# ChicyChen/LOCO-Edit

Measured on AMD Instinct MI355X. Metric: edit-directions/sec (top-5 PMP-Jacobian SVD @256^2) + vT cos-sim vs ref, higher is better.
Workload: dtype bf16x3 (split-bf16 MFMA operands, fp32 accumulate + fp32 storage); 1 GPU; CelebA-HQ DDPM 256x256 top-5 local basis (l_eye-sized mask, L=2400), t=0.6T, 12 power iterations, one GPU; multi_gpu_form=single, probes_total=5, probes_per_gpu=5, kept=5, n_iter=12, mask_L=2400, weights=synthetic seed 0, streams=2

## Files before the change

### loco-edit_amd/csrc/conv_bf16_kernel.h

```cpp
#pragma once
#include "kernels.h"
#include <cstdlib>
#include <type_traits>

namespace loco {


typedef float f32x16 __attribute__((ext_vector_type(16)));
typedef float f32x4 __attribute__((ext_vector_type(4)));
typedef f32x4 f32x4_u __attribute__((aligned(4)));
typedef float f32x2 __attribute__((ext_vector_type(2)));
typedef f32x2 f32x2_u __attribute__((aligned(4)));
typedef __bf16 bf16x8 __attribute__((ext_vector_type(8)));
typedef _Float16 f16x8 __attribute__((ext_vector_type(8)));
typedef short s16x8 __attribute__((ext_vector_type(8)));

enum : int { PR_BF16X3 = 0, PR_F16 = 1 };

constexpr int BKC = 16;
constexpr bool LIVE_MASK = true;
constexpr bool EARLY_W = true;
constexpr int NDUMMY = 8;

__device__ __forceinline__ float sigmoidf2_(float y) { return __builtin_amdgcn_rcpf(1.0f + __expf(-y)); }
// ... 46 lines not shown
    if (taps == 1) return NT;
    if (NT >= 128) {
        int th = NT / 32;
        return s2 ? (2 * th + 1) * 65 : (th + 2) * 34;
    }
    return s2 ? 5 * 65 : 4 * 34;
}

constexpr int rs_steps(int n, int lw) { int s = 0; while ((1 << s) < lw && (n >> s) > 1) ++s; return s; }
template <int N, int M, int LW>
__device__ __forceinline__ void rs_reduce(float* av, const int lane) {
    if constexpr (M < LW && N > 1) {
        constexpr int H = N / 2;
        const bool up = (lane & M) != 0;
#pragma unroll
        for (int i = 0; i < H; ++i) {
            const float keep = up ? av[i + H] : av[i];
            const float send = up ? av[i] : av[i + H];
            av[i] = keep + __shfl_xor(send, M, 64);
        }
        rs_reduce<H, M * 2, LW>(av, lane);
    } else if constexpr (M < LW) {
#pragma unroll
        for (int i = 0; i < N; ++i) av[i] += __shfl_xor(av[i], M, 64);
        rs_reduce<N, M * 2, LW>(av, lane);
    }
}

constexpr int EPI_COT1 = 1, EPI_STATS = 2;
template <int WM, int WN, int TM, int TN, int EPI = EPI_STATS, class StageRound>
__device__ __forceinline__ void conv_lowp_epilogue_staged(const ConvArgs& a, StageRound&& stage_round, unsigned char* smem_b, const int co0,
                                                          const int oy0, const int ox0, const int TW, const int tile_id, const int b,
                                                          const int split);
template <int WM, int WN, int TM, int TN>
__device__ __forceinline__ void conv_lowp_epilogue_direct(const ConvArgs& a, f32x16 (&acc)[TM][TN], const int co0, const int oy0,
                                                          const int ox0, const int TW, const int b, const int split);
template <int WM, int WN, int TM, int TN, int EPI = EPI_STATS>
__device__ __forceinline__ void conv_lowp_epilogue(const ConvArgs& a, f32x16 (&acc)[TM][TN], unsigned char* smem_b, const int co0,
                                                   const int oy0, const int ox0, const int TW, const int tile_id, const int b,
                                                   const int split) {
    constexpr int NT = WN * TN * 32;
    const int lane = threadIdx.x & 63, wave = threadIdx.x >> 6;
    const int l31 = lane & 31, khalf = lane >> 5, wm = wave / WN, wn = wave % WN;
    if (co0 + WM * TM * 32 <= a.Cout) {
        conv_lowp_epilogue_staged<WM, WN, TM, TN, EPI>(a, [&](const int h, float* S) {
#pragma unroll
            for (int j = 0; j < TN; ++j)
#pragma unroll
                for (int r = 0; r < 16; ++r)
                    S[(wm * 32 + (r & 3) + 8 * (r >> 2) + 4 * khalf) * NT + (wn * TN + j) * 32 + l31] = acc[h][j][r];
        }, smem_b, co0, oy0, ox0, TW, tile_id, b, split);
        return;
    }
    conv_lowp_epilogue_direct<WM, WN, TM, TN>(a, acc, co0, oy0, ox0, TW, b, split);
}
template <int WM, int WN, int TM, int TN, int EPI, class StageRound>
__device__ __forceinline__ void conv_lowp_epilogue_staged(const ConvArgs& a, StageRound&& stage_round, unsigned char* smem_b, const int co0,
                                                          const int oy0, const int ox0, const int TW, const int tile_id, const int b,
                                                          const int split) {
    constexpr int NTHR = WM * WN * 64;
    constexpr bool COT1 = (EPI & EPI_COT1) != 0, STATS = (EPI & EPI_STATS) != 0;
    constexpr int MT = WM * TM * 32;
    constexpr int NT = WN * TN * 32;
    const int tid = threadIdx.x;
    const int lane = tid & 63;
    const int wave = tid >> 6;
    const int l31 = lane & 31;
    const int khalf = lane >> 5;
    const int wm = wave / WN, wn = wave % WN;
    const long out_plane = (long)a.Hout * a.Wout;
    {
        constexpr int SROWS = WM * 32, NQ = NT / 4, NTASK = (SROWS * NQ) / NTHR;
        static_assert((SROWS * NQ) % NTHR == 0 && (NQ & (NQ - 1)) == 0, "epilogue task split");
        float* const S = reinterpret_cast<float*>(smem_b);
        const bool part = a.nsplit > 1;
        float* const ob = part ? a.partial + (((long)split * a.B + b) * a.Cout) * out_plane : a.out + (long)b * a.out_bs;
        const float* const rb = (!part && a.res) ? a.res + (long)b * a.res_bs : nullptr;
        const float* const b2 = (!part && a.bias2) ? a.bias2 + (long)b * a.bias2_bs : nullptr;
        const float* const b1 = part ? nullptr : a.bias;
        const bool accu = !part && a.accumulate;
        const int twsh = 31 - __builtin_clz((unsigned)TW);
        const bool lin_st = STATS && (a.st_kind == ST_TAN || a.st_kind == ST_COT) && !part;
        const bool lin_cot = a.st_kind == ST_COT;
        const bool cot_ep = COT1 && a.cot_d && !part && !lin_st;
        const float* const cot_db = cot_ep ? a.cot_d + (long)b * a.cot_d_bs : nullptr;
        const f32x2* const cot_tb = cot_ep ? reinterpret_cast<const f32x2*>(a.cot_tc + (long)b * a.cot_tc_bs) : nullptr;
        constexpr int RSTEP = NTHR / NQ;
// ... 110 lines not shown
                        s1 += __shfl_xor(s1, m, 64);
                        s2 += __shfl_xor(s2, m, 64);
                    }
                    const float m = s1 * (1.0f / NT);
                    const int t = q * NTHR + tid;
                    if ((t & (NQ - 1)) == 0)
                        *reinterpret_cast<f32x2*>(sp + ((long)co_of(h, q) * ntile + tile_id) * 2) = f32x2{pivot + m, s2 - s1 * m};
                }
            }
        }
        if constexpr (STATS) if (lin_st) {
            constexpr int LW = NQ < 64 ? NQ : 64, STEPS = rs_steps(NV, LW), LEFT = NV >> STEPS;
            static_assert((NV & (NV - 1)) == 0, "row sums per lane");
            rs_reduce<NV, 1, LW>(av, lane);
            const int gl = lane & (LW - 1);
            if (gl < (1 << STEPS)) {
                int base = 0;
#pragma unroll
                for (int sb = 0; sb < STEPS; ++sb) base += ((gl >> sb) & 1) * (NV >> (sb + 1));
                const int ntile = (a.Hout * a.Wout) / NT;
                float* const sp = a.st_part + (long)b * a.Cout * ntile * 2;
#pragma unroll
                for (int i = 0; i < LEFT; ++i) {
                    const int idx = base + i, hq = idx >> 1;
                    const int h = hq / NTASK, q = hq - h * NTASK;
                    const int row = (q * NTHR + tid) / NQ;
                    const int co = co0 + ((row >> 5) * TM + h) * 32 + (row & 31);
                    sp[((long)co * ntile + tile_id) * 2 + (idx & 1)] = av[i];
                }
            }
        }
    }
}
template <int WM, int WN, int TM, int TN>
__device__ __forceinline__ void conv_lowp_epilogue_direct(const ConvArgs& a, f32x16 (&acc)[TM][TN], const int co0, const int oy0,
                                                          const int ox0, const int TW, const int b, const int split) {
    const int lane = threadIdx.x & 63, wave = threadIdx.x >> 6;
    const int l31 = lane & 31, khalf = lane >> 5, wm = wave / WN, wn = wave % WN;
    const long out_plane = (long)a.Hout * a.Wout;
    const bool full_co = false;
#pragma unroll
    for (int j = 0; j < TN; ++j) {
        int p = (wn * TN + j) * 32 + l31;
        int ty = p / TW, tx = p - ty * TW;
        int oy = oy0 + ty, ox = ox0 + tx;
        const unsigned pix = (unsigned)(oy * a.Wout + ox);
#pragma unroll
        for (int i = 0; i < TM; ++i) {
            const int cob = co0 + (wm * TM + i) * 32 + 4 * khalf;
            if (a.nsplit > 1) {
                float* pb = a.partial + (((long)split * a.B + b) * a.Cout) * out_plane;
#pragma unroll
                for (int r = 0; r < 16; ++r) {
                    int co = cob + (r & 3) + 8 * (r >> 2);
                    if (full_co || co < a.Cout) pb[(long)co * out_plane + pix] = acc[i][j][r];
                }
            } else {
                float* ob = a.out + (long)b * a.out_bs;
                const float* rb = a.res ? a.res + (long)b * a.res_bs : nullptr;
                const float* b2 = a.bias2 ? a.bias2 + (long)b * a.bias2_bs : nullptr;
                if (rb || a.accumulate) {
                    float rv[16];
#pragma unroll
                    for (int r = 0; r < 16; ++r) {
                        int co = cob + (r & 3) + 8 * (r >> 2);
                        const bool ok = full_co || co < a.Cout;
                        const long off = (long)(ok ? co : a.Cout - 1) * out_plane + pix;
                        float t = 0.f;
                        if (rb) t = a.res_scale * rb[off];
                        if (a.accumulate) t += ob[off];
                        rv[r] = t;
                    }
#pragma unroll
                    for (int r = 0; r < 16; ++r) {
                        int co = cob + (r & 3) + 8 * (r >> 2);
                        if (!(full_co || co < a.Cout)) continue;
// ... 1 lines not shown
                        if (a.bias) v += a.bias[co];
                        if (b2) v += b2[co];
                        __builtin_nontemporal_store(v, &ob[(long)co * out_plane + pix]);
                    }
                } else {
#pragma unroll
                    for (int r = 0; r < 16; ++r) {
                        int co = cob + (r & 3) + 8 * (r >> 2);
                        if (!(full_co || co < a.Cout)) continue;
                        float v = acc[i][j][r];
                        if (a.bias) v += a.bias[co];
                        if (b2) v += b2[co];
                        __builtin_nontemporal_store(v, &ob[(long)co * out_plane + pix]);
                    }
                }
            }
        }
    }
}

template <int PR, int TAPS, int WM, int WN, int TM, int TN, int MODE, int STG, int PHASE = 0>
__device__ __forceinline__ void conv_lowp_body(const ConvArgs& a, f32x16 (&acc)[TM][TN]) {
    constexpr int NTHR = WM * WN * 64;
    constexpr int HP = halo_pitch<PR>();
    constexpr int RB = rec_bytes<PR>();
    constexpr int NPC = RB / 16;
    constexpr int MT = WM * TM * 32;
    constexpr int NT = WN * TN * 32;
    constexpr int KS = (TAPS == 9) ? 3 : 1;
    constexpr int NTS = KS;
    constexpr int NROW = (TAPS == 9) ? 3 : 1;
    constexpr bool NEEDP = (MODE == CM_TAN_SILU || MODE == CM_COT_SILU);
    constexpr bool GEN = (STG == 1 || STG == 2);
    constexpr int NITEM = GEN ? (2 * max_halo(NT, TAPS, STG == 2) + NTHR - 1) / NTHR : 1;
    constexpr int WTOT = NTS * MT * NPC;
    constexpr int NWV = (WTOT + NTHR - 1) / NTHR;
    constexpr bool XPF = (TAPS == 9 && STG != 2);
    constexpr int NWB = XPF ? 3 : 2;
    constexpr bool DEEP1 = (TAPS == 1 && STG == 1 && !NEEDP);
    constexpr int DEEP_D = 4;

    extern __shared__ __attribute__((aligned(16))) unsigned char smem_b[];
#ifdef LOCO_DUAL_STAMP
#define LP_STAMP(i) do { if (threadIdx.x == 0 && PHASE == 0) reinterpret_cast<unsigned long long*>(a.partial)[blockIdx.x * 8 + (i)] = __builtin_amdgcn_s_memtime(); } while (0)
#else
#define LP_STAMP(i) do { } while (0)
#endif
    LP_STAMP(0);
    constexpr int WBYTES = NTS * MT * RB;
    unsigned char* const Wsb = smem_b;
    unsigned char* Hsb;
    unsigned char* Ws = smem_b;
    unsigned char* Hs = smem_b;

    const int tid = threadIdx.x;
    const int lane = tid & 63;
    const int wave = tid >> 6;
    const int l31 = lane & 31;
    const int khalf = lane >> 5;
    const int wm = wave / WN, wn = wave % WN;

    const int S = a.stride;
    const int TW = (TAPS == 1 && PHASE == 0 && a.stride == 1 && !a.upsample && !a.zins && (a.Wout & (a.Wout - 1)) == 0)
                       ? (a.Wout < NT ? a.Wout : NT) : (a.Wout < 32 ? a.Wout : 32);
    const int TH = NT / TW;
    const int tiles_x = a.Wout / TW;
// ... 23 lines not shown
    const int co0 = cot_id * MT;
    int zb_, zs_;
    idivmod_small(zid, a.nsplit, zb_, zs_);
    const int b = __builtin_amdgcn_readfirstlane(zb_);
    const int split = __builtin_amdgcn_readfirstlane(zs_);

    if constexpr (XPF && PHASE != 2 && EARLY_W) {
        const int nchunks_ = (a.Cin + BKC - 1) / BKC;
        const int cps_ = __builtin_amdgcn_readfirstlane((nchunks_ + a.nsplit - 1) / a.nsplit);
        const int cbeg_ = split * cps_;
        const int cend_ = (cbeg_ + cps_ < nchunks_) ? cbeg_ + cps_ : nchunks_;
        if (cend_ > cbeg_) {
            typedef __attribute__((address_space(3))) unsigned char lds_u8_;
            typedef const __attribute__((address_space(1))) unsigned char glb_u8_;
            const int wpitch_ = (a.Cout + 31) & ~31;
            const unsigned char* wbase0 = reinterpret_cast<const unsigned char*>(a.wb) +
                                          (unsigned)(cbeg_ * TAPS) * ((unsigned)wpitch_ * (unsigned)RB);
#pragma unroll
            for (int st_ = 0; st_ < 2; ++st_)
#pragma unroll
                for (int i = 0; i < NWV; ++i) {
                    int e = tid + i * NTHR;
                    if (e >= WTOT) e = WTOT - 1;
                    const int tap = e / (MT * NPC), rem = e - tap * (MT * NPC);
                    int rec = co0 + rem / NPC;
                    if (rec >= wpitch_) rec = wpitch_ - 1;
                    const unsigned rel = (unsigned)(((st_ * NTS + tap) * wpitch_ + rec) * NPC + (rem % NPC)) * 16u;
                    const int e0 = wave * 64 + i * NTHR;
                    if ((WTOT % NTHR) == 0 || e0 < WTOT)
                        __builtin_amdgcn_global_load_lds((glb_u8_*)(wbase0 + rel), (lds_u8_*)(smem_b + st_ * WBYTES + e0 * 16), 16, 0, 0);
                }
        }
    }
    const int halo_w = (TW - 1) * S + KS;
    const int halo_h = (TH - 1) * S + KS;
    const int halo_sz = halo_h * halo_w;
    const int HBYTES = (halo_sz + NDUMMY) * HP;
    Hsb = smem_b + NWB * WBYTES;

    const int LH = (a.upsample || a.zins) ? a.Hin * 2 : a.Hin;
    const int LW = (a.upsample || a.zins) ? a.Win * 2 : a.Win;
    const long in_plane = (long)a.Hin * a.Win;

    int ipos[NITEM], ioct[NITEM];
    unsigned ivoff[NITEM];
    bool ival[NITEM];
#pragma unroll
    for (int i = 0; i < NITEM; ++i) {
        int it = tid + i * NTHR;
        int oct, pos;
        idivmod_small(it, halo_sz, oct, pos);
        int off = -1;
        if (it < 2 * halo_sz) {
            int hy, hx;
            idivmod_small(pos, halo_w, hy, hx);
            int Y = oy0 * S - a.pad + hy, X = ox0 * S - a.pad + hx;
            if (Y >= 0 && Y < LH && X >= 0 && X < LW) {
                if (a.upsample) off = (Y >> 1) * a.Win + (X >> 1);
                else if (a.zins) off = ((Y | X) & 1) ? -1 : (Y >> 1) * a.Win + (X >> 1);
                else off = Y * a.Win + X;
            }
        } else {
            pos = -1; oct = 0;
        }
        ipos[i] = pos; ioct[i] = oct;
        ival[i] = off >= 0;
        ivoff[i] = (unsigned)(oct * 8 * (int)in_plane + (off >= 0 ? off : 0));
    }

    const int nseg = (halo_w + 3) >> 2;
    int v_q4 = 0, v_pos0 = -1, v_voff = 0, v_cnt = 0;
    unsigned v_pm = 0;
    int v_rec[4] = {0, 0, 0, 0};
    unsigned v_goff = 0;
    if constexpr (!GEN) {
        const int per_q = halo_h * nseg;
        const int nsg4 = (nseg + 3) >> 2, nhy2 = (halo_h + 1) >> 1;
        bool have = false;
        int hy = 0, sg = 0;
        if (32 * nsg4 * nhy2 <= NTHR) {
            const int hi = tid >> 5;
            v_q4 = (tid >> 3) & 3;
            int hq_, hr_;
            idivmod_small(hi, nsg4, hq_, hr_);
            sg = hr_ * 4 + (tid & 3);
            hy = hq_ * 2 + ((tid >> 2) & 1);
            have = hi < nsg4 * nhy2 && sg < nseg && hy < halo_h;
            if (!have) v_q4 = 0;
        } else if (tid < 4 * per_q) {
            int rem;
            idivmod_small(tid, per_q, v_q4, rem);
            idivmod_small(rem, nseg, hy, sg);
            have = true;
        }
        if (have) {
            int Y = oy0 - a.pad + hy, X0 = ox0 - a.pad + 4 * sg;
            bool rowok = (Y >= 0 && Y < a.Hin);
            v_pos0 = hy * halo_w + 4 * sg;
            v_cnt = halo_w - 4 * sg < 4 ? halo_w - 4 * sg : 4;
            v_voff = rowok ? Y * a.Win + X0 : 0;
#pragma unroll
            for (int pxi = 0; pxi < 4; ++pxi)
                if (rowok && X0 + pxi >= 0 && X0 + pxi < a.Win && pxi < v_cnt) v_pm |= 1u << pxi;
        }
#pragma unroll
        for (int pxi = 0; pxi < 4; ++pxi)
            v_rec[pxi] = (v_pos0 >= 0 && pxi < v_cnt) ? v_pos0 + pxi : halo_sz + (tid & (NDUMMY - 1));
        v_goff = (unsigned)(((long)v_q4 * 4 * in_plane + v_voff + 16) * 4);
    }

    int hoff[TN];
#pragma unroll
    for (int j = 0; j < TN; ++j) {
        int p = (wn * TN + j) * 32 + l31;
        int ty, tx;
        idivmod_small(p, TW, ty, tx);
        hoff[j] = ty * S * halo_w + tx * S;
    }
    int hbyte[TN];
#pragma unroll
    for (int j = 0; j < TN; ++j) hbyte[j] = hrec_off<PR>(hoff[j], khalf);
    int aoff_hi[TM], aoff_lo[TM];
#pragma unroll
    for (int i = 0; i < TM; ++i) {
        int p = (wm * TM + i) * 32 + l31;
        aoff_hi[i] = rec_off<PR>(p, khalf);
        aoff_lo[i] = PR == PR_F16 ? 0 : rec_off<PR>(p, 2 + khalf);
    }

    if constexpr (PHASE != 2) {
#pragma unroll
        for (int i = 0; i < TM; ++i)
#pragma unroll
            for (int j = 0; j < TN; ++j)
#pragma unroll
                for (int r = 0; r < 16; ++r) acc[i][j][r] = 0.0f;
    }

    const int nchunks = (a.Cin + BKC - 1) / BKC;
    const int cps = __builtin_amdgcn_readfirstlane((nchunks + a.nsplit - 1) / a.nsplit);
    const int cbeg = split * cps;
    const int cend = (cbeg + cps < nchunks) ? cbeg + cps : nchunks;

    const float* inb = a.in + (long)b * a.in_bs;
    const float2* sxb = NEEDP ? a.sx : nullptr;
    const float* scb = (MODE == CM_GN_SILU || MODE == CM_GN || MODE == CM_GN_GELU) ? a.sc + (long)b * a.scsh_bs : nullptr;
    const float* shb = (MODE == CM_GN_SILU || MODE == CM_GN || MODE == CM_GN_GELU) ? a.sh + (long)b * a.scsh_bs : nullptr;
    const int wpitch = (a.Cout + 31) & ~31;
    const uint4* wg = reinterpret_cast<const uint4*>(a.wb);

// ... 294 lines not shown
#elif defined(LOCO_WI_2MFMA)
            acc[i][j] = __builtin_amdgcn_mfma_f32_32x32x16_bf16(ah, bl, acc[i][j], 0, 0, 0);
            acc[i][j] = __builtin_amdgcn_mfma_f32_32x32x16_bf16(ah, bh, acc[i][j], 0, 0, 0);
            (void)al;
            return;
#endif
            acc[i][j] = __builtin_amdgcn_mfma_f32_32x32x16_bf16(al, bh, acc[i][j], 0, 0, 0);
            acc[i][j] = __builtin_amdgcn_mfma_f32_32x32x16_bf16(ah, bl, acc[i][j], 0, 0, 0);
            acc[i][j] = __builtin_amdgcn_mfma_f32_32x32x16_bf16(ah, bh, acc[i][j], 0, 0, 0);
        }
    };
    auto mma_frag_head = [&](const Frag& f) { mma_one(f, 0, 0); };
    auto mma_frag_tail = [&](const Frag& f) {
#pragma unroll
        for (int i = 0; i < TM; ++i)
#pragma unroll
            for (int j = 0; j < TN; ++j)
                if (i + j > 0) mma_one(f, i, j);
    };

    const int nch = cend - cbeg;
    const int clast = cend - 1;
    auto cclamp = [&](int c) { return __builtin_amdgcn_readfirstlane(c < clast ? c : clast); };
    auto vres = [&](int x) -> int {
        if (x <= clast) { pf_live = true; return __builtin_amdgcn_readfirstlane(x); }
        pf_live = !LIVE_MASK;
        return clast;
    };
    auto stage_end = [&]() {
        asm volatile("s_waitcnt lgkmcnt(0)" ::: "memory");
        __builtin_amdgcn_s_barrier();
        asm volatile("" ::: "memory");
    };
    if constexpr (XPF) {
        Frag fr[2];
        auto stage_of = [&](int ci_, int row_, int& c_out, int& r_out) {
            c_out = cclamp(cbeg + ci_ + row_ / NROW);
            r_out = row_ % NROW;
        };
        LP_STAMP(1);
        if (nch > 0) {
            if constexpr (!(PHASE != 2 && EARLY_W)) {
                int c1, r1;
                dma_w(cbeg, 0, Wsb);
                stage_of(0, 1, c1, r1);
                dma_w(c1, r1, Wsb + WBYTES);
            }
            Hs = Hsb;
            if constexpr (!GEN && NPART == 2) {
                HaloRegs hr2;
                prefetch_hv(hr, cbeg, 0);
                prefetch_hv(hr2, cbeg, 1);
                stage_hv(hr, 0);
                stage_hv(hr2, 1);
            } else {
                prefetch_h(cbeg, 0);
                stage_h(cbeg, 0);
            }
            asm volatile("s_waitcnt vmcnt(0)" ::: "memory");
            prefetch_h(cclamp(cbeg + 1), 0);
            stage_end();
            Ws = Wsb; Hs = Hsb;
            load_frag(fr[0], 0, 0);
        }
        LP_STAMP(2);
        auto chunk_body = [&](auto ptag, const int ci) {
            constexpr int P = decltype(ptag)::value;
// ... 179 lines not shown
            Ws = Wcur; Hs = Hcur;
            Frag f0, f1;
            load_frag(f0, row, 0);
            if (NTS > 1) load_frag(f1, row, 1);
            __builtin_amdgcn_sched_barrier(0);
            mma_frag(f0);
            __builtin_amdgcn_sched_barrier(0);
            if (NTS > 2) load_frag(f0, row, 2);
            __builtin_amdgcn_sched_barrier(0);
            if (NTS > 1) mma_frag(f1);
            if (st_part >= 0) { Hs = Hnxt; stage_h(cclamp(chunk + 1), st_part); Hs = Hcur; }
            if (MIDLOAD && ld_part >= 0) { pf_live = LIVE_MASK ? (ld_chunk <= clast) : true; prefetch_h(cclamp(ld_chunk), ld_part); pf_live = true; }
            if (NTS > 2) mma_frag(f0);
            __builtin_amdgcn_sched_barrier(0);
            if (MIDLOAD && ld_part >= 0) {
                asm volatile("s_waitcnt vmcnt(%0)" :: "n"(NLD) : "memory");
            } else {
                asm volatile("s_waitcnt vmcnt(0)" ::: "memory");
                if (!MIDLOAD && ld_part >= 0) { pf_live = LIVE_MASK ? (ld_chunk <= clast) : true; prefetch_h(cclamp(ld_chunk), ld_part); pf_live = true; }
            }
            stage_end();
        }
    }
    }

    }

    if constexpr (PHASE == 1) {
        asm volatile("s_waitcnt lgkmcnt(0)" ::: "memory");
        __builtin_amdgcn_s_barrier();
        return;
    }
    LP_STAMP(3);
    conv_lowp_epilogue<WM, WN, TM, TN, (TAPS == 1 && PHASE == 0) ? (EPI_COT1 | EPI_STATS) : EPI_STATS>(a, acc, smem_b, co0, oy0, ox0, TW, tile_id, b, split);
    LP_STAMP(4);
#undef LP_STAMP
}

constexpr int lowp_min_waves(int taps, int nthr) { return (taps == 1 && nthr <= 256) ? 2 : 1; }
template <int TAPS, int WM, int WN, int TM, int TN, int MODE, int STG>
__global__ __launch_bounds__(WM * WN * 64, lowp_min_waves(TAPS, WM * WN * 64)) void conv_mfma_bf16x3(ConvArgs a) {
    f32x16 acc[TM][TN];
    conv_lowp_body<PR_BF16X3, TAPS, WM, WN, TM, TN, MODE, STG>(a, acc);
}
template <int TAPS, int WM, int WN, int TM, int TN, int MODE, int STG>
__global__ __launch_bounds__(WM * WN * 64, lowp_min_waves(TAPS, WM * WN * 64)) void conv_mfma_f16(ConvArgs a) {
    f32x16 acc[TM][TN];
    conv_lowp_body<PR_F16, TAPS, WM, WN, TM, TN, MODE, STG>(a, acc);
}

template <int PR, int WM, int WN, int TM, int TN, int MODE>
__device__ __forceinline__ void conv_lowp_kcat(const ConvArgs& a) {
    f32x16 acc[TM][TN];
    conv_lowp_body<PR, 9, WM, WN, TM, TN, MODE, 0, 1>(a, acc);
    ConvArgs a2 = a;
    a2.in = a.in2; a2.in_bs = a.in2_bs; a2.Cin = a.Cin2; a2.wb = a.wb2; a2.mode = CM_NONE; a2.pad = 0; a2.in_padded = a.in2_padded;
    conv_lowp_body<PR, 1, WM, WN, TM, TN, CM_NONE, 1, 2>(a2, acc);
}
template <int WM, int WN, int TM, int TN, int MODE>
__global__ __launch_bounds__(WM * WN * 64) void conv_kcat_bf16x3(ConvArgs a) { conv_lowp_kcat<PR_BF16X3, WM, WN, TM, TN, MODE>(a); }
template <int WM, int WN, int TM, int TN, int MODE>
__global__ __launch_bounds__(WM * WN * 64) void conv_kcat_f16(ConvArgs a) { conv_lowp_kcat<PR_F16, WM, WN, TM, TN, MODE>(a); }

template <int PR, int TAPS, int WM, int WN, int TM, int TN, int MODE, int STG>
static void launch_one_b2(const ConvArgs& a, hipStream_t st) {
    constexpr int MT = WM * TM * 32, NT = WN * TN * 32;
    constexpr int KS = (TAPS == 9) ? 3 : 1;
    int TW = a.Wout < 32 ? a.Wout : 32;
    int TH = NT / TW;
    int halo_w = (TW - 1) * a.stride + KS, halo_h = (TH - 1) * a.stride + KS;
    const int nwb = (TAPS == 9 && STG != 2) ? 3 : 2;
    size_t lds = (size_t)nwb * KS * MT * rec_bytes<PR>() + 2 * ((size_t)halo_w * halo_h + NDUMMY) * halo_pitch<PR>();
    const size_t stage_bytes = (size_t)WM * 32 * NT * 4;
    if (lds < stage_bytes) lds = stage_bytes;
    dim3 grid(((a.Hout * a.Wout) / NT) * ((a.Cout + MT - 1) / MT) * a.B * a.nsplit);
    void (*kern)(ConvArgs);
    if constexpr (PR == PR_F16) kern = &conv_mfma_f16<TAPS, WM, WN, TM, TN, MODE, STG>;
    else kern = &conv_mfma_bf16x3<TAPS, WM, WN, TM, TN, MODE, STG>;
    if (lds > 64 * 1024) {
        static DeviceOnce once;
        if (first_on_device(once)) {
            (void)hipFuncSetAttribute(reinterpret_cast<const void*>(kern), hipFuncAttributeMaxDynamicSharedMemorySize,
                                      160 * 1024);
        }
    }
    hipLaunchKernelGGL(kern, grid, dim3(WM * WN * 64), lds, st, a);
}

template <int PR, int TAPS, int WM, int WN, int TM, int TN, int MODE>
static void launch_one_b(const ConvArgs& a, hipStream_t st) {
    const bool general = a.stride != 1 || a.upsample || a.zins || (a.Cin % BKC) != 0 || !a.in_padded;
    if constexpr (MODE == CM_NONE) {
        if (a.stride == 2) launch_one_b2<PR, TAPS, WM, WN, TM, TN, MODE, 2>(a, st);
        else if (TAPS == 9 && !general) launch_one_b2<PR, TAPS, WM, WN, TM, TN, MODE, 0>(a, st);
        else launch_one_b2<PR, TAPS, WM, WN, TM, TN, MODE, 1>(a, st);
        return;
    }
    if constexpr (MODE == CM_GN_SILU || MODE == CM_TAN_SILU || MODE == CM_GN_GELU) {
        if (general) { launch_one_b2<PR, TAPS, WM, WN, TM, TN, MODE, 1>(a, st); return; }
    }
    launch_one_b2<PR, TAPS, WM, WN, TM, TN, MODE, 0>(a, st);
}


template <int PR, int MODE>
void launch_kcat_b(const ConvArgs& a, hipStream_t st) {
    constexpr int WM = 2, WN = 4, TM = 2, TN = 2, MT = 128, NT = 256;
    const int TW = a.Wout < 32 ? a.Wout : 32, TH = NT / TW;
    size_t lds = (size_t)3 * 3 * MT * rec_bytes<PR>() + 2 * ((size_t)(TW + 2) * (TH + 2) + NDUMMY) * halo_pitch<PR>();
    dim3 grid(((a.Hout * a.Wout) / NT) * ((a.Cout + MT - 1) / MT) * a.B * a.nsplit);
    void (*kern)(ConvArgs);
    if constexpr (PR == PR_F16) kern = &conv_kcat_f16<WM, WN, TM, TN, MODE>;
    else kern = &conv_kcat_bf16x3<WM, WN, TM, TN, MODE>;
    static DeviceOnce once;
    if (first_on_device(once))
        (void)hipFuncSetAttribute(reinterpret_cast<const void*>(kern), hipFuncAttributeMaxDynamicSharedMemorySize, 160 * 1024);
    hipLaunchKernelGGL(kern, grid, dim3(WM * WN * 64), lds, st, a);
}

template <int PR, int TAPS, int MODE>
void launch_tile_b(const ConvArgs& a, hipStream_t st) {
    switch (a.tile) {
        case 5:
            launch_one_b<PR, TAPS, 2, 4, 2, 2, MODE>(a, st);
            break;
// ... 10 lines not shown
```

### loco-edit_amd/csrc/conv_plan.hip

```cpp
#include "kernels.h"
#include <cstdio>
#include <cstdlib>

namespace loco {

constexpr int BKC = 16;
constexpr int BKF = 8;

static const int kMT[6] = {128, 128, 32, 64, 128, 128}, kNT[6] = {128, 64, 128, 64, 256, 256};

static int env_int(const char* name, int dflt) {
    const char* e = getenv(name);
    return e ? atoi(e) : dflt;
}
static int pick_tile(int Cout, int HW) {
    if (HW >= 128) return Cout > 32 ? 0 : 2;
    return Cout > 64 ? 1 : 3;
}

static int conv_pick_nsplit(int Cin, int Cout, int Hout, int Wout, int B) {
    const int t = pick_tile(Cout, Hout * Wout);
    long blocks = (long)((Hout * Wout) / kNT[t]) * ((Cout + kMT[t] - 1) / kMT[t]) * B;
    int nchunks = (Cin + BKF - 1) / BKF;
    if (blocks >= 384 || nchunks < 8) return 1;
// ... 35 lines not shown
    if (t == 4) t = 5;
    if (taps == 1 && t == 5 && B >= 2 && HW <= kTile0MaxHW) t = 0;
    long blocks = (long)(HW / kNT[t]) * ((Cout + kMT[t] - 1) / kMT[t]) * B;
    int nchunks = (Cin + BKC - 1) / BKC;
    int target = chip_share > 1 ? 256 / chip_share : (lanes == 2 ? 240 : 256);
    if (target < 32) target = 32;
    if (blocks >= target / 2 || nchunks < 8) return 1;
    int want = (int)(target / blocks);
    int maxs = nchunks / 4;
    if (want > maxs) want = maxs;
    if (want > 32) want = 32;
    return want < 1 ? 1 : want;
}

static bool conv_lowp_can_kcat(const ConvArgs& a) {
    static const bool on = env_int("LOCO_KCAT", 1) != 0;
    return on && a.Cin2 > 0 && a.nsplit == 1 && bf16_tile_of(a) == 5 && a.stride == 1 && !a.upsample && !a.zins && a.pad == 1 &&
           (a.Cin % BKC) == 0 && (a.Cin2 % BKC) == 0 && a.in_padded &&
           (a.mode == CM_GN_SILU || a.mode == CM_GN_GELU || a.mode == CM_TAN_SILU);
}
static bool conv_lowp_can_fuse_stats(const ConvArgs& a) {
    return a.nsplit <= 1 && !a.gemm && (a.Cout % conv_bf16_tile_couts(a)) == 0;
}

static bool conv_pair_ok(const ConvArgs& a) {
    static const bool on = env_int("LOCO_CONV_PAIR", 1) != 0;
    if (!on || a.Hout * a.Wout < 16384 || a.taps != 9 || a.Cin2 > 0 || a.nsplit != 1 || a.stride != 1 || a.upsample || a.zins ||
        a.pad != 1 || !a.in_padded || (a.Cin % (2 * BKC)) != 0 || (a.Cout % 128) != 0 || (a.Wout % 32) != 0 || (a.Hout % 8) != 0)
        return false;
    if (!(a.mode == CM_NONE || a.mode == CM_GN_SILU || a.mode == CM_TAN_SILU || a.mode == CM_COT_SILU)) return false;
    return a.tile == 5;
}

static ConvArgs conv_shift_batch(const ConvArgs& a, int nb) {
    ConvArgs t = a;
    t.B = a.B - nb;
    t.in += (long)nb * a.in_bs; t.out += (long)nb * a.out_bs;
    if (t.prim) t.prim += (long)nb * a.prim_bs;
    if (t.bias2) t.bias2 += (long)nb * a.bias2_bs;
    if (t.res) t.res += (long)nb * a.res_bs;
    if (t.sc) { t.sc += (long)nb * a.scsh_bs; t.sh += (long)nb * a.scsh_bs; }
    if (t.mr) t.mr += (long)nb * a.mr_bs;
    if (t.tst) t.tst += (long)nb * a.tst_bs;
    if (t.tc) t.tc += (long)nb * a.tc_bs;
    if (t.in2) t.in2 += (long)nb * a.in2_bs;
    if (t.cot_d) { t.cot_d += (long)nb * a.cot_d_bs; t.cot_tc += (long)nb * a.cot_tc_bs; }
    if (t.st_part) t.st_part += (long)nb * a.Cout * ((a.Hout * a.Wout) / conv_bf16_tile_pixels(a)) * 2;
    return t;
}

static void conv_gemm_plan(ConvArgs& a) {
    static const bool on = env_int("LOCO_CONV_GEMM", 1) != 0;
    a.gemm = 0;
    const long HW = (long)a.Hout * a.Wout;
    if (!on || a.stride != 1 || a.upsample || a.zins || (a.Cin % BKC) != 0 || a.Cin < 320 || (HW % 256) != 0 || (a.Wout % 16) != 0 ||
        a.Cout < 128 || !a.partial || a.Cin2 > 0 || !(a.mode == CM_NONE || a.mode == CM_GN) || a.cot_d)
        return;
    {
        const int TW = a.Wout < 32 ? a.Wout : 32;
        if ((256 % TW) != 0 || (a.Wout % TW) != 0 || (a.Hout % (256 / TW)) != 0) return;
    }
    static const int all_shapes = env_int("LOCO_GEMM_ALL", 0);
    if (!all_shapes && !(a.Cout >= 640 && (a.Cout >= 4 * a.Cin || a.Cin >= 2560))) return;
    const int pad256 = (a.Cout + 255) / 256 * 256;
    const int tm = (pad256 * 10 <= a.Cout * 11) ? 4 : 2;
    const int mt = 64 * tm;
    const long tiles = (HW / 256) * ((a.Cout + mt - 1) / mt) * a.B;
    const size_t rec_floats = (size_t)a.B * a.Cin * HW;
    int ns = 1;
    if (tiles < 192) {
        const int nchunks = a.Cin / BKC;
        ns = (int)((256 + tiles - 1) / tiles);
        if (ns > 8) ns = 8;
        while (ns > 1 && nchunks / ns < 8) --ns;
        while (ns > 1 && (size_t)ns * a.B * a.Cout * HW + rec_floats > a.partial_floats) --ns;
    }
    if ((ns > 1 ? (size_t)ns * a.B * a.Cout * HW : 0) + rec_floats > a.partial_floats) return;
    a.gemm = 1; a.gemm_tm = tm; a.nsplit = ns;
}

void conv_plan_family(ConvArgs& a, int prec) {
    if (prec == 1 && a.taps == 1) conv_gemm_plan(a);
}

void conv_plan_tile_pair(ConvArgs& a, int prec, int tile_override) {
    a.tile = tile_for(a, prec, tile_override);
    a.pair = prec == 1 && conv_pair_ok(a);
}

static bool short_tail(long per_probe, int B) {
    const long total = per_probe * B, r = total % 256;
    return total > 256 && r > 0 && r <= 160;
}

static int tail_split(const ConvArgs& a, size_t partial_floats, int* split) {
    const long per_probe = (long)((a.Hout * a.Wout) / conv_bf16_tile_pixels(a)) * ((a.Cout + 127) / 128);
    const long r = per_probe * a.B % 256;
    if (!short_tail(per_probe, a.B) || per_probe <= 0 || r % per_probe != 0 || r / per_probe >= a.B) return 0;
    int s = (int)(256 / r);
    if (s > 4) s = 4;
    const int nchunks = (a.Cin + 15) / 16;
    while (s > 1 && nchunks / s < 4) --s;
    const size_t one = (size_t)(r / per_probe) * a.Cout * a.Hout * a.Wout;
    while (s > 1 && (size_t)s * one > partial_floats) --s;
    *split = s;
    return s > 1 ? (int)(r / per_probe) : 0;
}

static int stats_route(const ConvEnv& e, const StatAsk* q, bool want, ConvArgs& x, int s0, int B, int* keep_ntile) {
    if (!q || q->kind == ST_NONE) return SR_NONE;
    const int alone = q->norm ? SR_ALONE : SR_NONE;
    if (!want) return alone;
    if (x.nsplit > 1) return !q->norm ? SR_NONE : ((x.Hout * x.Wout) % 4 == 0 ? SR_SPLITK : SR_ALONE);
    const int ntile = (x.Hout * x.Wout) / conv_bf16_tile_pixels(x);
    const size_t need = (size_t)x.B * x.Cout * ntile * 2;
    const int epi = q->norm ? SR_EPI : SR_KEEP;
    const bool kept = q->keep && s0 == 0 && x.B == B && need <= q->keep_floats;
    if (q->kind == ST_FWD && conv_lowp_can_fuse_stats(x) && (kept || (q->norm && need <= e.stpart_floats))) {
        x.st_part = kept ? q->keep : e.stpart; x.st_kind = ST_FWD;
        if (kept) *keep_ntile = ntile;
// ... 54 lines not shown
        const long per_probe = (long)((a.Hout * a.Wout) / conv_bf16_tile_pixels(t)) * ((a.Cout + 127) / 128);
        p.cot = e.prec >= 1 && taps == 1 && a.nsplit == 1 && !short_tail(per_probe, a.B) && conv_lowp_can_fuse_stats(t);
        if (!p.cot) { a.cot_d = nullptr; a.cot_d_bs = 0; a.cot_sx = nullptr; a.cot_tc = nullptr; a.cot_tc_bs = 0; }
    }
    while (a.nsplit > 1 && (size_t)a.nsplit * a.B * a.Cout * a.Hout * a.Wout > e.partial_floats) a.nsplit >>= 1;
    if (a.nsplit < 1) a.nsplit = 1;
    a.partial = e.partial;
    a.partial_floats = e.partial_floats;
    conv_plan_family(a, e.prec);
    a.tile = tile_for(a, e.prec, -1);
    int split = 1;
    const int tail = e.prec >= 1 && a.nsplit == 1 && a.B >= 2 && !a.gemm ? tail_split(a, e.partial_floats, &split) : 0;
    const bool want = q && q->kind != ST_NONE && e.prec >= 1 && e.fuse_stats;
    if (!tail) {
        p.l[0] = plan_launch(e, q, want, a, 0, a.B, &p.keep_ntile);
        return p;
    }
    const bool per_part = want && q->norm && (q->kind == ST_FWD || (e.fuse_lin && (a.Hout * a.Wout) % 4 == 0));
    p.stats_all = !per_part && q && q->kind != ST_NONE && q->norm;
    const StatAsk* ql = per_part ? q : nullptr;
    const int nb = a.B - tail;
    ConvArgs m = a, t = conv_shift_batch(a, nb);
    m.B = nb;
    t.nsplit = split;
    p.nl = 2;
    p.l[0] = plan_launch(e, ql, want, m, 0, a.B, &p.keep_ntile);
    p.l[1] = plan_launch(e, ql, want, t, nb, a.B, &p.keep_ntile);
    return p;
}

const char* conv_variant_name(const ConvArgs& a, int taps, int prec) {
    static const char* tiles[6] = {"2,2,2,2", "4,1,1,2", "1,4,1,1", "2,2,1,1", "2,2,2,4", "2,4,2,2"};
    static char names[3][2][6][6][56];
    static char others[3][3][6][40];
    const int mode = (a.mode < 0 || a.mode > 5) ? 2 : a.mode;
    const char* other = nullptr;
    int k = 0, v = mode;
    if (prec && taps == 9 && a.Cin2 > 0) other = prec == 1 ? "conv_kcat_bf16x3<2,4,2,2,%d>" : "conv_kcat_f16<2,4,2,2,%d>";
    else if (prec == 1 && taps == 1 && a.gemm) { k = 1; other = "conv_gemm_bf16x3<%d>"; v = a.gemm_tm; }
    else if (prec == 1 && taps == 9 && a.pair) { k = 2; other = "conv_pair_bf16x3<%d>"; }
    if (other) {
        char* n = others[k][prec][v];
        if (!n[0]) snprintf(n, 40, other, v);
        return n;
    }
    int t = a.tile;
    if (t < 0 || t > 5) t = 0;
    int m = mode;
    if (taps != 9 && m != CM_NONE) m = CM_GN;
    if (!prec && m == CM_GN_GELU) m = CM_GN_SILU;
    char* n = names[prec][taps == 9 ? 0 : 1][t][m];
    static const char* kn[3] = {"conv_mfma_f32", "conv_mfma_bf16x3", "conv_mfma_f16"};
    if (!n[0]) snprintf(n, 56, "%s<%d,%s,%d>", kn[prec], taps, tiles[t], m);
    return n;
}

}
```

### loco-edit_amd/csrc/conv_plan_text.h

```cpp
#pragma once
#include "kernels.h"
#include <cstdio>
#include <string>

namespace loco {

inline void conv_plan_text(const ConvPlan& p, int taps, int prec, std::string& out) {
    char line[320];
    for (int li = 0; li < p.nl; ++li) {
        const ConvLaunch& l = p.l[li];
        const ConvArgs& y = l.args;
        snprintf(line, sizeof(line),
                 "launch=%d part=0 kernel=%s tile=%d nsplit=%d B=%d s0=%d gemm=%d gemm_tm=%d pair=%d Cin2=%d sc_first=%d cot=%d\n",
                 li, conv_variant_name(y, taps, prec), y.tile, y.nsplit, y.B, l.s0, y.gemm, y.gemm ? y.gemm_tm : 0, y.pair, y.Cin2,
                 p.sc_first ? 1 : 0, p.cot ? 1 : 0);
        out += line;
    }
}

}
```

### loco-edit_amd/csrc/kernels.h

```cpp
#pragma once
#include <hip/hip_runtime.h>
#include <stdint.h>

namespace loco {

struct DeviceOnce { bool seen[64] = {}; };
inline bool first_on_device(DeviceOnce& f) {
    int d = 0;
    (void)hipGetDevice(&d);
    d &= 63;
    if (f.seen[d]) return false;
    f.seen[d] = true;
    return true;
}


enum ConvMode : int {
    CM_NONE = 0,
    CM_GN_SILU = 1,
    CM_GN = 2,
    CM_TAN_SILU = 3,
    CM_COT_SILU = 4,
    CM_GN_GELU = 5,
};
// ... 19 lines not shown
    const float2* sx;
    float* out; long out_bs; int Cout, Hout, Wout;
    const float* bias;
    const float* bias2; long bias2_bs;
    const float* res; long res_bs;
    const float* sc; const float* sh; long scsh_bs;
    const float* mr; long mr_bs;
    const float* gamma_;
    const float* tst; long tst_bs;
    const float* tc; long tc_bs;
    int cpg;
    int mode;
    int stride;
    int pad;
    int upsample;
    int zins;
    int in_padded;
    int accumulate;
    int nsplit;
    int taps;
    int no_deep;
    float* partial;
    int B;
    float* st_part; int st_kind;
    const float* st_x; const float2* st_sx;
    const float* in2; long in2_bs; int Cin2; int in2_padded;
    const void* wb2;
    const float* cot_d; long cot_d_bs; const float2* cot_sx; const float* cot_tc; long cot_tc_bs;
    int act;
    float res_scale;
    int gemm, gemm_tm;
    size_t partial_floats;
    int tile, pair;
};

void launch_conv(const ConvArgs& a, int taps, hipStream_t st);
void launch_conv_bf16x3(const ConvArgs& a, int taps, hipStream_t st);
void launch_conv_f16(const ConvArgs& a, int taps, hipStream_t st);
void launch_conv_splitk_reduce(const ConvArgs& a, hipStream_t st);

struct ConvEnv {
    int prec = 1;
    int chip_share = 1;
    int lanes = 1, lane_s0 = 0;
    float* partial = nullptr; size_t partial_floats = 0;
    float* stpart = nullptr; size_t stpart_floats = 0;
    bool fuse_stats = true, fuse_lin = true, deep1 = true;
    int max_batch = 1;
};

struct StatAsk {
    int kind = ST_NONE;
    bool norm = false;
    const float2* sx = nullptr;
    const float* prim = nullptr;
    float* keep = nullptr; size_t keep_floats = 0;
};

enum StatRoute : int {
    SR_NONE = 0,
    SR_EPI = 1,
    SR_SPLITK = 2,
    SR_ALONE = 3,
    SR_KEEP = 4,
};

// ... 182 lines not shown
```

Measured before the change: 19.68 edit-directions/s.

## Add phase-sorted zero-insertion conv path that skips MMAs on inserted zeros

Adds a specialised STG=3 conv body for zero-inserted (transposed/upsampling) 3x3 convolutions. It stages only the real input pixels into a compact halo and groups output pixels by sub-pixel phase, so each wave issues only the one or two kernel taps per row that touch non-zero inputs. The epilogue gets a pixel-mapping functor to scatter the phase-sorted results. This is meant to remove the MFMA work and halo traffic spent multiplying inserted zeros, at the cost of a complex hand-scheduled pipeline limited to one tile shape and a narrow set of conditions.

New measurement: 19.81 edit-directions/s, median of 6. No clear change (+0.7%).

```diff
diff --git a/loco-edit_amd/csrc/conv_bf16_kernel.h b/loco-edit_amd/csrc/conv_bf16_kernel.h
--- a/loco-edit_amd/csrc/conv_bf16_kernel.h
+++ b/loco-edit_amd/csrc/conv_bf16_kernel.h
@@ -102,27 +102,35 @@
 __device__ __forceinline__ void conv_lowp_epilogue_staged(const ConvArgs& a, StageRound&& stage_round, unsigned char* smem_b, const int co0,
                                                           const int oy0, const int ox0, const int TW, const int tile_id, const int b,
                                                           const int split);
-template <int WM, int WN, int TM, int TN>
-__device__ __forceinline__ void conv_lowp_epilogue_direct(const ConvArgs& a, f32x16 (&acc)[TM][TN], const int co0, const int oy0,
+template <int WM, int WN, int TM, int TN, class PixOf>
+__device__ __forceinline__ void conv_lowp_epilogue_direct(const ConvArgs& a, f32x16 (&acc)[TM][TN], PixOf&& pix_of, const int co0, const int oy0,
                                                           const int ox0, const int TW, const int b, const int split);
+template <int WM, int WN, int TM, int TN, int EPI = EPI_STATS, class PixOf>
+__device__ __forceinline__ void conv_lowp_epilogue(const ConvArgs& a, f32x16 (&acc)[TM][TN], PixOf&& pix_of, unsigned char* smem_b, const int co0,
+                                                   const int oy0, const int ox0, const int TW, const int tile_id, const int b,
+                                                   const int split) {
+    constexpr int NT = WN * TN * 32;
+    const int lane = threadIdx.x & 63, wave = threadIdx.x >> 6;
+    const int khalf = lane >> 5, wm = wave / WN;
+    if (co0 + WM * TM * 32 <= a.Cout) {
+        conv_lowp_epilogue_staged<WM, WN, TM, TN, EPI>(a, [&](const int h, float* S) {
+#pragma unroll
+            for (int j = 0; j < TN; ++j)
+#pragma unroll
+                for (int r = 0; r < 16; ++r)
+                    S[(wm * 32 + (r & 3) + 8 * (r >> 2) + 4 * khalf) * NT + pix_of(j)] = acc[h][j][r];
+        }, smem_b, co0, oy0, ox0, TW, tile_id, b, split);
+        return;
+    }
+    conv_lowp_epilogue_direct<WM, WN, TM, TN>(a, acc, pix_of, co0, oy0, ox0, TW, b, split);
+}
 template <int WM, int WN, int TM, int TN, int EPI = EPI_STATS>
 __device__ __forceinline__ void conv_lowp_epilogue(const ConvArgs& a, f32x16 (&acc)[TM][TN], unsigned char* smem_b, const int co0,
                                                    const int oy0, const int ox0, const int TW, const int tile_id, const int b,
                                                    const int split) {
-    constexpr int NT = WN * TN * 32;
-    const int lane = threadIdx.x & 63, wave = threadIdx.x >> 6;
-    const int l31 = lane & 31, khalf = lane >> 5, wm = wave / WN, wn = wave % WN;
-    if (co0 + WM * TM * 32 <= a.Cout) {
-        conv_lowp_epilogue_staged<WM, WN, TM, TN, EPI>(a, [&](const int h, float* S) {
-#pragma unroll
-            for (int j = 0; j < TN; ++j)
-#pragma unroll
-                for (int r = 0; r < 16; ++r)
-                    S[(wm * 32 + (r & 3) + 8 * (r >> 2) + 4 * khalf) * NT + (wn * TN + j) * 32 + l31] = acc[h][j][r];
-        }, smem_b, co0, oy0, ox0, TW, tile_id, b, split);
-        return;
-    }
-    conv_lowp_epilogue_direct<WM, WN, TM, TN>(a, acc, co0, oy0, ox0, TW, b, split);
+    const int l31 = threadIdx.x & 31, wn = (threadIdx.x >> 6) % WN;
+    conv_lowp_epilogue<WM, WN, TM, TN, EPI>(a, acc, [&](const int j) -> int { return (wn * TN + j) * 32 + l31; }, smem_b, co0, oy0, ox0, TW,
+                                            tile_id, b, split);
 }
 template <int WM, int WN, int TM, int TN, int EPI, class StageRound>
 __device__ __forceinline__ void conv_lowp_epilogue_staged(const ConvArgs& a, StageRound&& stage_round, unsigned char* smem_b, const int co0,
@@ -299,16 +307,16 @@
         }
     }
 }
-template <int WM, int WN, int TM, int TN>
-__device__ __forceinline__ void conv_lowp_epilogue_direct(const ConvArgs& a, f32x16 (&acc)[TM][TN], const int co0, const int oy0,
+template <int WM, int WN, int TM, int TN, class PixOf>
+__device__ __forceinline__ void conv_lowp_epilogue_direct(const ConvArgs& a, f32x16 (&acc)[TM][TN], PixOf&& pix_of, const int co0, const int oy0,
                                                           const int ox0, const int TW, const int b, const int split) {
     const int lane = threadIdx.x & 63, wave = threadIdx.x >> 6;
-    const int l31 = lane & 31, khalf = lane >> 5, wm = wave / WN, wn = wave % WN;
+    const int khalf = lane >> 5, wm = wave / WN;
     const long out_plane = (long)a.Hout * a.Wout;
     const bool full_co = false;
 #pragma unroll
     for (int j = 0; j < TN; ++j) {
-        int p = (wn * TN + j) * 32 + l31;
+        int p = pix_of(j);
         int ty = p / TW, tx = p - ty * TW;
         int oy = oy0 + ty, ox = ox0 + tx;
         const unsigned pix = (unsigned)(oy * a.Wout + ox);
@@ -376,6 +384,9 @@
     constexpr int NROW = (TAPS == 9) ? 3 : 1;
     constexpr bool NEEDP = (MODE == CM_TAN_SILU || MODE == CM_COT_SILU);
     constexpr bool GEN = (STG == 1 || STG == 2);
+    constexpr bool ZS = (STG == 3);
+    static_assert(!ZS || (TAPS == 9 && MODE == CM_NONE && PHASE == 0 && WM == 2 && WN == 4 && TM == 2 && TN == 2), "phase-sorted zero-insertion tile");
+    constexpr int ZS_HW = 32, ZS_VW = 17, ZS_HH = 5;
     constexpr int NITEM = GEN ? (2 * max_halo(NT, TAPS, STG == 2) + NTHR - 1) / NTHR : 1;
     constexpr int WTOT = NTS * MT * NPC;
     constexpr int NWV = (WTOT + NTHR - 1) / NTHR;
@@ -465,9 +476,11 @@
                 }
         }
     }
-    const int halo_w = (TW - 1) * S + KS;
-    const int halo_h = (TH - 1) * S + KS;
+    const int halo_w = ZS ? ZS_HW : (TW - 1) * S + KS;
+    const int halo_vw = ZS ? ZS_VW : halo_w;
+    const int halo_h = ZS ? ZS_HH : (TH - 1) * S + KS;
     const int halo_sz = halo_h * halo_w;
+    const int hy_org = ZS ? (oy0 - a.pad + 1) >> 1 : oy0 - a.pad, hx_org = ZS ? (ox0 - a.pad + 1) >> 1 : ox0 - a.pad;
     const int HBYTES = (halo_sz + NDUMMY) * HP;
     Hsb = smem_b + NWB * WBYTES;
 
@@ -501,7 +514,7 @@
         ivoff[i] = (unsigned)(oct * 8 * (int)in_plane + (off >= 0 ? off : 0));
     }
 
-    const int nseg = (halo_w + 3) >> 2;
+    const int nseg = (halo_vw + 3) >> 2;
     int v_q4 = 0, v_pos0 = -1, v_voff = 0, v_cnt = 0;
     unsigned v_pm = 0;
     int v_rec[4] = {0, 0, 0, 0};
@@ -527,10 +540,11 @@
             have = true;
         }
         if (have) {
-            int Y = oy0 - a.pad + hy, X0 = ox0 - a.pad + 4 * sg;
+            int Y = hy_org + hy, X0 = hx_org + 4 * sg;
             bool rowok = (Y >= 0 && Y < a.Hin);
+            if constexpr (ZS) rowok = rowok && X0 < a.Win;
             v_pos0 = hy * halo_w + 4 * sg;
-            v_cnt = halo_w - 4 * sg < 4 ? halo_w - 4 * sg : 4;
+            v_cnt = halo_vw - 4 * sg < 4 ? halo_vw - 4 * sg : 4;
             v_voff = rowok ? Y * a.Win + X0 : 0;
 #pragma unroll
             for (int pxi = 0; pxi < 4; ++pxi)
@@ -549,6 +563,30 @@
         int ty, tx;
         idivmod_small(p, TW, ty, tx);
         hoff[j] = ty * S * halo_w + tx * S;
+    }
+    const int zh = ZS ? __builtin_amdgcn_readfirstlane(wn >> 1) : 0, zg = ZS ? __builtin_amdgcn_readfirstlane(wn & 1) : 0;
+    int zs_kxa[3] = {0, 0, 0}, zs_toa[3] = {0, 0, 0}, zs_tob[3] = {0, 0, 0}, zpix[TN];
+    bool zs_two[3] = {false, false, false};
+#pragma unroll
+    for (int j = 0; j < TN; ++j) zpix[j] = 0;
+    if constexpr (ZS) {
+        const int pr = a.pad & 1;
+#pragma unroll
+        for (int j = 0; j < TN; ++j) {
+            const int ry = j, rx = j ? 1 - zh : zh;
+            hoff[j] = (2 * zg + (l31 >> 4)) * halo_w + (l31 & 15);
+            zpix[j] = (2 * (2 * zg + (l31 >> 4)) + (ry ^ pr)) * 32 + 2 * (l31 & 15) + (rx ^ pr);
+        }
+#pragma unroll
+        for (int ky = 0; ky < 3; ++ky) {
+            const int j = ky & 1, ry = j, rx = j ? 1 - zh : zh;
+            const int rys = pr ? -ry : ry, rxs = pr ? -rx : rx;
+            zs_two[ky] = rx == 0;
+            zs_kxa[ky] = zs_two[ky] ? 0 : 1;
+            const int dy = (rys + ky) >> 1;
+            zs_toa[ky] = dy * halo_w + ((rxs + zs_kxa[ky]) >> 1);
+            zs_tob[ky] = dy * halo_w + ((rxs + 2) >> 1);
+        }
     }
     int hbyte[TN];
 #pragma unroll
@@ -909,7 +947,94 @@
         __builtin_amdgcn_s_barrier();
         asm volatile("" ::: "memory");
     };
-    if constexpr (XPF) {
+    if constexpr (ZS) {
+        struct ZFrag { s16x8 ah[TM], al[NLO ? TM : 1], bh, bl; };
+        auto zs_load = [&](ZFrag& f, const unsigned char* Wb, const unsigned char* Hb, const int kx, const int toff, const int j) {
+#pragma unroll
+            for (int i = 0; i < TM; ++i) {
+                f.ah[i] = *reinterpret_cast<const s16x8*>(Wb + kx * MT * RB + aoff_hi[i]);
+                if constexpr (NLO) f.al[i] = *reinterpret_cast<const s16x8*>(Wb + kx * MT * RB + aoff_lo[i]);
+            }
+            const unsigned char* hp = Hb + toff * HP + hbyte[j];
+            f.bh = *reinterpret_cast<const s16x8*>(hp);
+            if constexpr (NLO) f.bl = *reinterpret_cast<const s16x8*>(hp + 32);
+        };
+        auto zs_mma = [&](const ZFrag& f, const int j) {
+#pragma unroll
+            for (int i = 0; i < TM; ++i) {
+                if constexpr (PR == PR_F16) {
+                    acc[i][j] = __builtin_amdgcn_mfma_f32_32x32x16_f16(__builtin_bit_cast(f16x8, f.ah[i]), __builtin_bit_cast(f16x8, f.bh),
+                                                                       acc[i][j], 0, 0, 0);
+                } else {
+                    const bf16x8 ah = __builtin_bit_cast(bf16x8, f.ah[i]), al = __builtin_bit_cast(bf16x8, f.al[i]);
+                    const bf16x8 bh = __builtin_bit_cast(bf16x8, f.bh), bl = __builtin_bit_cast(bf16x8, f.bl);
+                    acc[i][j] = __builtin_amdgcn_mfma_f32_32x32x16_bf16(al, bh, acc[i][j], 0, 0, 0);
+                    acc[i][j] = __builtin_amdgcn_mfma_f32_32x32x16_bf16(ah, bl, acc[i][j], 0, 0, 0);
+                    acc[i][j] = __builtin_amdgcn_mfma_f32_32x32x16_bf16(ah, bh, acc[i][j], 0, 0, 0);
+                }
+            }
+        };
+        static_assert(NPART == 2 && NROW == 3 && XPF, "vector staging in two parts, three weight buffers");
+        ZFrag za[2], zb;
+        if (nch > 0) {
+            if constexpr (!EARLY_W) {
+                dma_w(cbeg, 0, Wsb);
+                dma_w(cbeg, 1, Wsb + WBYTES);
+            }
+            Hs = Hsb;
+            HaloRegs hr2;
+            prefetch_hv(hr, cbeg, 0);
+            prefetch_hv(hr2, cbeg, 1);
+            stage_hv(hr, 0);
+            stage_hv(hr2, 1);
+            asm volatile("s_waitcnt vmcnt(0)" ::: "memory");
+            prefetch_h(cclamp(cbeg + 1), 0);
+            stage_end();
+            zs_load(za[0], Wsb, Hsb, zs_kxa[0], zs_toa[0], 0);
+        }
+        auto zs_chunk = [&](auto ptag, const int ci) {
+            constexpr int P = decltype(ptag)::value;
+            const int chunk = cbeg + ci;
+            unsigned char* const Hcur = Hsb + P * HBYTES;
+            unsigned char* const Hnxt = Hsb + (1 - P) * HBYTES;
+#pragma unroll
+            for (int row = 0; row < NROW; ++row) {
+                unsigned char* const Wcur = Wsb + row * WBYTES;
+                unsigned char* const Wnx1 = Wsb + ((row + 1) % 3) * WBYTES;
+                unsigned char* const Wnx2 = Wsb + ((row + 2) % 3) * WBYTES;
+                const int nrow = (row + 1) % NROW, j = row & 1;
+                {
+                    const int x = chunk + (row + 2) / NROW;
+                    int c2;
+                    if (x <= clast) { c2 = x; dma_live = true; }
+                    else { c2 = clast; dma_live = !LIVE_MASK; }
+                    dma_w(__builtin_amdgcn_readfirstlane(c2), (row + 2) % NROW, Wnx2);
+                    dma_live = true;
+                }
+                ZFrag& fa = za[(P + row) & 1];
+                ZFrag& fn = za[(P + row + 1) & 1];
+                if (zs_two[row]) zs_load(zb, Wcur, Hcur, 2, zs_tob[row], j);
+                __builtin_amdgcn_sched_barrier(0);
+                if (row == 2) { const int cx = vres(chunk + 2); prefetch_h(cx, 0); pf_live = true; }
+                zs_mma(fa, j);
+                __builtin_amdgcn_sched_barrier(0);
+                zs_load(fn, Wnx1, row + 1 < NROW ? Hcur : Hnxt, zs_kxa[nrow], zs_toa[nrow], nrow & 1);
+                __builtin_amdgcn_sched_barrier(0);
+                if (row == 0) { Hs = Hnxt; stage_h(cclamp(chunk + 1), 0); }
+                if (zs_two[row]) zs_mma(zb, j);
+                if (row == 1) { Hs = Hnxt; stage_h(cclamp(chunk + 1), 1); }
+                if (row == 0) { const int cx = vres(chunk + 1); prefetch_h(cx, 1); pf_live = true; }
+                __builtin_amdgcn_sched_barrier(0);
+                if (row != 1) asm volatile("s_waitcnt vmcnt(%0)" :: "n"(KP) : "memory");
+                else asm volatile("s_waitcnt vmcnt(0)" ::: "memory");
+                stage_end();
+            }
+        };
+        for (int ci = 0; ci < nch; ci += 2) {
+            zs_chunk(std::integral_constant<int, 0>{}, ci);
+            if (ci + 1 < nch) zs_chunk(std::integral_constant<int, 1>{}, ci + 1);
+        }
+    } else if constexpr (XPF) {
         Frag fr[2];
         auto stage_of = [&](int ci_, int row_, int& c_out, int& r_out) {
             c_out = cclamp(cbeg + ci_ + row_ / NROW);
@@ -1155,7 +1280,8 @@
         return;
     }
     LP_STAMP(3);
-    conv_lowp_epilogue<WM, WN, TM, TN, (TAPS == 1 && PHASE == 0) ? (EPI_COT1 | EPI_STATS) : EPI_STATS>(a, acc, smem_b, co0, oy0, ox0, TW, tile_id, b, split);
+    if constexpr (ZS) conv_lowp_epilogue<WM, WN, TM, TN, EPI_STATS>(a, acc, [&](const int j) -> int { return zpix[j]; }, smem_b, co0, oy0, ox0, TW, tile_id, b, split);
+    else conv_lowp_epilogue<WM, WN, TM, TN, (TAPS == 1 && PHASE == 0) ? (EPI_COT1 | EPI_STATS) : EPI_STATS>(a, acc, smem_b, co0, oy0, ox0, TW, tile_id, b, split);
     LP_STAMP(4);
 #undef LP_STAMP
 }
@@ -1192,6 +1318,7 @@
     int TW = a.Wout < 32 ? a.Wout : 32;
     int TH = NT / TW;
     int halo_w = (TW - 1) * a.stride + KS, halo_h = (TH - 1) * a.stride + KS;
+    if (STG == 3) { halo_w = 32; halo_h = 5; }
     const int nwb = (TAPS == 9 && STG != 2) ? 3 : 2;
     size_t lds = (size_t)nwb * KS * MT * rec_bytes<PR>() + 2 * ((size_t)halo_w * halo_h + NDUMMY) * halo_pitch<PR>();
     const size_t stage_bytes = (size_t)WM * 32 * NT * 4;
@@ -1214,6 +1341,9 @@
 static void launch_one_b(const ConvArgs& a, hipStream_t st) {
     const bool general = a.stride != 1 || a.upsample || a.zins || (a.Cin % BKC) != 0 || !a.in_padded;
     if constexpr (MODE == CM_NONE) {
+        if constexpr (TAPS == 9 && WM == 2 && WN == 4 && TM == 2 && TN == 2) {
+            if (a.zskip) { launch_one_b2<PR, TAPS, WM, WN, TM, TN, MODE, 3>(a, st); return; }
+        }
         if (a.stride == 2) launch_one_b2<PR, TAPS, WM, WN, TM, TN, MODE, 2>(a, st);
         else if (TAPS == 9 && !general) launch_one_b2<PR, TAPS, WM, WN, TM, TN, MODE, 0>(a, st);
         else launch_one_b2<PR, TAPS, WM, WN, TM, TN, MODE, 1>(a, st);
diff --git a/loco-edit_amd/csrc/conv_plan.hip b/loco-edit_amd/csrc/conv_plan.hip
--- a/loco-edit_amd/csrc/conv_plan.hip
+++ b/loco-edit_amd/csrc/conv_plan.hip
@@ -91,6 +91,13 @@
     return a.tile == 5;
 }
 
+static bool conv_zskip_ok(const ConvArgs& a, int prec) {
+    static const bool on = env_int("LOCO_ZINS_SKIP", 1) != 0;
+    return on && prec >= 1 && a.zins && !a.upsample && a.stride == 1 && a.taps == 9 && a.mode == CM_NONE && a.nsplit == 1 && a.tile == 5 &&
+           !a.pair && !a.gemm && a.Cin2 == 0 && (a.pad == 1 || a.pad == 2) && a.Wout >= 32 && (a.Wout % 32) == 0 && (a.Hout % 8) == 0 &&
+           a.Hout == 2 * a.Hin && a.Wout == 2 * a.Win && (a.Cin % BKC) == 0 && a.in_padded;
+}
+
 static ConvArgs conv_shift_batch(const ConvArgs& a, int nb) {
     ConvArgs t = a;
     t.B = a.B - nb;
@@ -145,6 +152,7 @@
 void conv_plan_tile_pair(ConvArgs& a, int prec, int tile_override) {
     a.tile = tile_for(a, prec, tile_override);
     a.pair = prec == 1 && conv_pair_ok(a);
+    a.zskip = conv_zskip_ok(a, prec);
 }
 
 static bool short_tail(long per_probe, int B) {
@@ -265,13 +273,16 @@
 const char* conv_variant_name(const ConvArgs& a, int taps, int prec) {
     static const char* tiles[6] = {"2,2,2,2", "4,1,1,2", "1,4,1,1", "2,2,1,1", "2,2,2,4", "2,4,2,2"};
     static char names[3][2][6][6][56];
-    static char others[3][3][6][40];
+    static char others[4][3][6][40];
     const int mode = (a.mode < 0 || a.mode > 5) ? 2 : a.mode;
     const char* other = nullptr;
     int k = 0, v = mode;
     if (prec && taps == 9 && a.Cin2 > 0) other = prec == 1 ? "conv_kcat_bf16x3<2,4,2,2,%d>" : "conv_kcat_f16<2,4,2,2,%d>";
     else if (prec == 1 && taps == 1 && a.gemm) { k = 1; other = "conv_gemm_bf16x3<%d>"; v = a.gemm_tm; }
     else if (prec == 1 && taps == 9 && a.pair) { k = 2; other = "conv_pair_bf16x3<%d>"; }
+    else if (prec && taps == 9 && a.zskip) {
+        k = 3; other = prec == 1 ? "conv_mfma_bf16x3<9,2,4,2,2,%d,zskip>" : "conv_mfma_f16<9,2,4,2,2,%d,zskip>";
+    }
     if (other) {
         char* n = others[k][prec][v];
         if (!n[0]) snprintf(n, 40, other, v);
diff --git a/loco-edit_amd/csrc/conv_plan_text.h b/loco-edit_amd/csrc/conv_plan_text.h
--- a/loco-edit_amd/csrc/conv_plan_text.h
+++ b/loco-edit_amd/csrc/conv_plan_text.h
@@ -11,9 +11,9 @@
         const ConvLaunch& l = p.l[li];
         const ConvArgs& y = l.args;
         snprintf(line, sizeof(line),
-                 "launch=%d part=0 kernel=%s tile=%d nsplit=%d B=%d s0=%d gemm=%d gemm_tm=%d pair=%d Cin2=%d sc_first=%d cot=%d\n",
+                 "launch=%d part=0 kernel=%s tile=%d nsplit=%d B=%d s0=%d gemm=%d gemm_tm=%d pair=%d Cin2=%d sc_first=%d cot=%d zskip=%d\n",
                  li, conv_variant_name(y, taps, prec), y.tile, y.nsplit, y.B, l.s0, y.gemm, y.gemm ? y.gemm_tm : 0, y.pair, y.Cin2,
-                 p.sc_first ? 1 : 0, p.cot ? 1 : 0);
+                 p.sc_first ? 1 : 0, p.cot ? 1 : 0, y.zskip);
         out += line;
     }
 }
diff --git a/loco-edit_amd/csrc/kernels.h b/loco-edit_amd/csrc/kernels.h
--- a/loco-edit_amd/csrc/kernels.h
+++ b/loco-edit_amd/csrc/kernels.h
@@ -75,6 +75,7 @@
     int gemm, gemm_tm;
     size_t partial_floats;
     int tile, pair;
+    int zskip;
 };
 
 void launch_conv(const ConvArgs& a, int taps, hipStream_t st);
```
